# hoivb612/neural

Measured on AMD Instinct MI355X. Metric: decode tokens/sec + prefill TFLOPS, Llama-2-7B int4-g128 at 1/2/4/8 MI355X, higher is better.
Workload: dtype f16; 1 GPU; Llama-2-7B int4-g128 sym decode linear stack, M=1 (32 x [QKV, O, gate/up+SiLU*mul, down] + lm_head), fp32 activations; group_size=128, batch=1, tp=1, parallelism=tp1, hip_graph=True

## Files before the change

neural_amd/bestla.py:

```python
import ctypes as C

import numpy as np

from ._lib import check, last_error, lib

F32, F16, BF16 = 32, 16, 16 | (1 << 16)
S8, S4, S2 = 8 | 0x100, 4 | 0x100, 2 | 0x100
COMP_UNDEF, COMP_F32, COMP_BF16, COMP_F16, COMP_INT8 = 0, 1, 2, 3, 4
ACT_F32, ACT_F16, ACT_BF16 = 0, 1, 2
EPI_NONE, EPI_BIAS, EPI_SILU_MUL, EPI_GELU_MUL, EPI_GELU, EPI_ADD_GELU, EPI_SILU, EPI_RES_ADD = range(8)

S1, S3, S5, S6, S7 = 1 | 0x100, 3 | 0x100, 5 | 0x100, 6 | 0x100, 7 | 0x100
F4_E2M1, F4_BNB, F4_NF4 = 4, 4 | (1 << 16), 4 | (2 << 16)
F8_E4M3, F8_E5M2, F8_E8M0 = 8, 8 | (1 << 16), 8 | (3 << 16)
DQ8_BNB = 8 | (4 << 16)
_WEIGHT_DTYPES = {"int4": S4, "int8": S8, "int2": S2, "int1": S1, "int3": S3, "int5": S5, "int6": S6, "int7": S7,
                  "fp4_e2m1": F4_E2M1, "fp4": F4_E2M1, "nf4": F4_NF4, "fp4_bnb": F4_BNB,
                  "fp8_e4m3": F8_E4M3, "fp8": F8_E4M3, "fp8_e5m2": F8_E5M2}
_SCALE_DTYPES = {"fp32": F32, "bf16": BF16, "fp16": F16, "fp8": F8_E8M0}
_COMP = {"int8": COMP_INT8, "bf16": COMP_BF16, "fp16": COMP_F16, "fp32": COMP_F32, "auto": COMP_UNDEF}
BITS = {S4: 4, S2: 2, S8: 8, S1: 1, S3: 3, S5: 5, S6: 6, S7: 7, F4_E2M1: 4, F4_BNB: 4, F4_NF4: 4, F8_E4M3: 8, F8_E5M2: 8}


def _ptr(a):
# ... 91 lines not shown
    return out


def split(blob, axis, rank, world, unit=1):
    L = lib()
    size = L.nad_blob_split(_ptr(blob), axis, rank, world, unit, None, 0)
    if not size:
        raise RuntimeError(f"nad_blob_split failed: {last_error()}")
    out = _aligned_buffer(size)
    if L.nad_blob_split(_ptr(blob), axis, rank, world, unit, _ptr(out), size) != size:
        raise RuntimeError(f"nad_blob_split failed: {last_error()}")
    return out


def split_range(blob, axis, rank, world, unit=1):
    b, e = C.c_int(0), C.c_int(0)
    check(lib().nad_split_range(_ptr(blob), axis, rank, world, unit, C.byref(b), C.byref(e)), "nad_split_range")
    return b.value, e.value


KERNELS = {1: "woq_gemv_m1_kernel", 2: "woq_gemv_kernel", 3: "woq_skinny_kernel", 4: "woq_i8_kernel",
           5: "woq_gemm3_kernel", 6: "woq_gemm4_kernel", 7: "woq_gemm2_kernel", 8: "woq_gemm_kernel",
           9: "woq_gemm7_kernel", 10: "woq_mid_kernel"}


def plan_forward(bits, n, k, group_size=128, scale_dtype="fp16", asym=False, m=1, act="fp32"):
    o = np.zeros(6, np.int64)
    st = {"fp32": 0, "bf16": 1, "fp16": 2}[scale_dtype]
    at = {"fp32": 0, "fp16": 1, "bf16": 2}[act]
    r = lib().nad_plan_forward(bits, n, k, group_size, st, int(asym), m, at, _ptr(o), 6)
    if r != 6:
        raise RuntimeError(f"nad_plan_forward failed: {last_error()}")
    return dict(kernel=KERNELS.get(int(o[0]), str(int(o[0]))), grid=int(o[1]), threads=int(o[2]), ksplit=int(o[3]),
                fold=bool(o[4] & 1), ksw=bool(o[4] & 2), launches=int(o[5]))


def _torch():
    import torch
    if not torch.cuda.is_available():
        raise RuntimeError("neural_amd device ops need a ROCm GPU (torch.cuda.is_available() is False)")
    return torch


def _stream(stream=None):
    torch = _torch()
    s = stream if stream is not None else torch.cuda.current_stream()
    return C.c_void_p(s.cuda_stream)


_ACT = {}


def _act_code(t):
    torch = _torch()
    if not _ACT:
        _ACT.update({torch.float32: ACT_F32, torch.float16: ACT_F16, torch.bfloat16: ACT_BF16})
    if t.dtype not in _ACT:
        raise TypeError(f"activation dtype {t.dtype} not supported (float32/float16/bfloat16)")
    return _ACT[t.dtype]


class DeviceWeight:

    def __init__(self, blob=None, device=None, stream=None, _desc=None, _mem=None):
        torch = _torch()
        L = lib()
        self.desc = (C.c_uint8 * L.bestla_device_storage_size())()
# ... 49 lines not shown
            raise RuntimeError(last_error())
        blocks = np.ascontiguousarray(blocks, dtype=np.uint8)
        assert blocks.size == n * (k // 32) * bb, (blocks.size, n, k, bb)
        need = L.nad_gguf_device_size(int(type), n, k)
        if not need:
            raise RuntimeError(last_error())
        mem = torch.empty(need, dtype=torch.uint8, device=device or "cuda")
        desc = (C.c_uint8 * L.bestla_device_storage_size())()
        check(L.nad_gguf_device_load(int(type), _ptr(blocks), n, k, desc, _ptr(mem), need, _stream(stream)),
              "nad_gguf_device_load")
        return cls(_desc=desc, _mem=mem)

    def forward(self, x, out=None, epilogue=EPI_NONE, bias=None, residual=None, stream=None):
        torch = _torch()
        m, k = x.shape
        assert k == self.k, (k, self.k)
        if out is None:
            out = torch.empty((m, self.n), dtype=torch.float32, device=x.device)
        bias_ld = 0 if bias is None or bias.dim() == 1 else bias.stride(0)
        check(lib().nad_device_forward(_ptr(x), _act_code(x), self.desc, _ptr(out), m, self.n, k, x.stride(0),
                                       out.stride(0), epilogue, _ptr(bias), bias_ld, _ptr(residual),
                                       residual.stride(0) if residual is not None else 0, _stream(stream)),
              "nad_device_forward")
        return out

    __call__ = forward

    def plan(self, m, act="fp32"):
        o = np.zeros(6, np.int64)
        at = {"fp32": 0, "fp16": 1, "bf16": 2}[act]
        if lib().nad_plan_weight(self.desc, m, at, _ptr(o), 6) != 6:
            raise RuntimeError(f"nad_plan_weight failed: {last_error()}")
        return dict(kernel=KERNELS.get(int(o[0]), str(int(o[0]))), grid=int(o[1]), threads=int(o[2]),
                    ksplit=int(o[3]), fold=bool(o[4] & 1), ksw=bool(o[4] & 2), launches=int(o[5]))

    def set_compute(self, mode):
        check(lib().nad_device_set_compute(self.desc, -1 if mode is None else int(mode)), "nad_device_set_compute")
        return self

    @property
    def compute(self):
        return lib().nad_device_get_compute(self.desc)

    def unpack(self, stream=None):
        out = np.zeros((self.k, self.n), np.float32)
        check(lib().nad_device_unpack_fp32(self.desc, _ptr(out), _stream(stream)), "nad_device_unpack_fp32")
        return out


COMPUTE_FP, COMPUTE_INT8 = 0, 1
GGUF_Q4_0, GGUF_Q4_1, GGUF_Q5_0, GGUF_Q5_1, GGUF_Q8_0 = 2, 3, 6, 7, 8


def set_compute_mode(mode):
    L = lib()
    prev = L.nad_get_compute_mode()
    check(L.nad_set_compute_mode(int(mode)), "nad_set_compute_mode")
    return prev


def get_compute_mode():
    return lib().nad_get_compute_mode()


def set_thread_compute_mode(mode):
    check(lib().nad_set_thread_compute_mode(-1 if mode is None else int(mode)), "nad_set_thread_compute_mode")

# ... 115 lines not shown
```

neural_amd/csrc/capi.hip:

```cpp
#include <hip/hip_runtime.h>

#include <atomic>
#include <cmath>
#include <climits>
#include <cstdarg>
#include <cstdio>
#include <cstdlib>
#include <cstring>
#include <mutex>
#include <string>
#include <unordered_map>
#include <vector>

#include "../../include/neural_amd.h"
#include "btla_format.h"
#include "woq_kernels.h"

using namespace nad;

static thread_local std::string g_err;
static void set_err(const char* fmt, ...) {
  char buf[512];
  va_list ap;
  va_start(ap, fmt);
  vsnprintf(buf, sizeof(buf), fmt, ap);
  va_end(ap);
  g_err = buf;
}
static void report(const char* where) { fprintf(stderr, "neural_amd: %s: %s\n", where, g_err.c_str()); }
#define HIP_OK(expr)                                                           \
  do {                                                                         \
    hipError_t e_ = (expr);                                                    \
    if (e_ != hipSuccess) {                                                    \
      set_err("%s failed: %s", #expr, hipGetErrorString(e_));                  \
      return -1;                                                               \
    }                                                                          \
  } while (0)

extern "C" const char* nad_last_error(void) { return g_err.c_str(); }
extern "C" void nad_clear_error(void) { g_err.clear(); }

static int env_int(const char* name, int def) {
  const char* v = getenv(name);
  return (v && *v) ? atoi(v) : def;
}

struct Knobs {
  int gemv_grid, gemv_waves, gemv_lean, gemv_spw, gemv_disable, gemv_dual, gemv_nst;
  int compute_int8;
  int gemm2_disable, gemm4_all, gemm4_disable, ffn_f32, gemm_kernel, gemm7_bm, splitk_disable;
  int gemm3_stagger, gemm4_fold_all, gemm4_fold, gemm4_ksw;
  int mid_min_m, mid_max_m, mid_ks, mid_xcd, mid_wide, gemm_xcd, gemm7_model, gemm7_fuse;
  int host_cache_mb;
};
static Knobs read_knobs() {
  Knobs k{};
  k.gemv_grid = env_int("NAD_GEMV_GRID", 0);
  k.gemv_waves = env_int("NAD_GEMV_WAVES", 0);
  k.gemv_nst = env_int("NAD_GEMV_NST", 0);
  k.gemv_lean = env_int("NAD_GEMV_LEAN", 1);
  k.gemv_dual = env_int("NAD_GEMV_DUAL", 1);
  k.gemv_spw = env_int("NAD_GEMV_SPW", 4);
  k.gemv_disable = env_int("NAD_GEMV_DISABLE", 0);
  k.compute_int8 = env_int("NAD_COMPUTE_INT8", 0);
  k.gemm2_disable = env_int("NAD_GEMM2_DISABLE", 0);
  k.gemm4_all = env_int("NAD_GEMM4_ALL", 0);
  k.gemm4_disable = env_int("NAD_GEMM4_DISABLE", 0);
  k.ffn_f32 = env_int("NAD_FFN_F32", 0);
  k.gemm_kernel = env_int("NAD_GEMM_KERNEL", 7);
  k.gemm7_bm = env_int("NAD_GEMM7_BM", 0);
  k.splitk_disable = env_int("NAD_SPLITK_DISABLE", 0);
  k.gemm3_stagger = env_int("NAD_GEMM3_STAGGER", 1);
  k.gemm4_fold_all = env_int("NAD_GEMM4_FOLD_ALL", 1);
  k.gemm4_fold = env_int("NAD_GEMM4_FOLD", 1);
  k.gemm4_ksw = env_int("NAD_GEMM4_KSW", 2);
  k.mid_max_m = env_int("NAD_MID_MAX_M", 64);
  k.mid_ks = env_int("NAD_MID_KS", 0);
  k.mid_xcd = env_int("NAD_MID_XCD", 1);
  k.mid_wide = env_int("NAD_MID_WIDE", 2);
  k.gemm_xcd = env_int("NAD_GEMM_XCD", 1);
  k.gemm7_fuse = env_int("NAD_GEMM7_FUSE", 1);
  k.gemm7_model = env_int("NAD_GEMM7_MODEL", 2);
  k.mid_min_m = env_int("NAD_MID_MIN_M", 0);
  k.host_cache_mb = env_int("NAD_HOST_CACHE_MB", 64 * 1024);
  return k;
}
static Knobs g_knobs = read_knobs();
static const Knobs& knobs() { return g_knobs; }
extern "C" void nad_reload_knobs(void) { g_knobs = read_knobs(); }

struct NadPlan {
  int kernel = 0, grid = 0, block = 0, ksplit = 1, fold = 0, launches = 0;
};
// ... 329 lines not shown
  a.act_t = act_t;
  a.dual = (epi == kEpiSiluMul || epi == kEpiGeluMul) ? 1 : 0;
  a.nt = w0.nt;
  a.ng = w0.ng;
  a.bs = w0.blocksize;
  a.tpg_mask = tpg == 0 ? 0x7fffffff : tpg - 1;
  a.tpg_shift = tpg == 0 ? 31 : __builtin_ctz(unsigned(tpg));
  a.scale_t = w0.scale_t;
  a.asym = w0.asym;
  a.epi = epi;
  a.shuffle = w0.shuffle;
  a.a_fast = (vec_aligned(act, lda, act_t) && w0.shuffle == nullptr && k % 8 == 0) ? 1 : 0;
  a.res = res;
  a.ld_res = ld_res;
  a.aux = aux;
  a.ld_aux = ld_aux;
  int stripes = 0;
  for (int i = 0; i < 4; i++) a.stripe_base[i] = INT_MAX;
  for (int i = 0; i < nw; i++) {
    a.w[i] = view(*ws[i], outs[i], ldos[i], bias, bias_ld);
    a.stripe_base[i] = stripes;
    stripes += ws[i]->ns;
  }
  for (int i = nw; i < 3; i++) a.w[i] = a.w[0];
  a.units = a.dual ? ws[0]->ns : stripes;
  const Knobs& kn = knobs();
  grid = std::max(1, std::min(a.units, device_cus()));
  if (kn.gemv_grid > 0) grid = std::min(a.units, kn.gemv_grid);
  waves = gemv_waves(w0.bits, w0.nt, w0.ng, w0.blocksize);
  if (kn.gemv_waves > 0) waves = std::min(gpt > 1 ? 8 : 16, kn.gemv_waves);
  a.dq_mask = 0x000F000Fu;
  a.dq_magic = 0x64006400u;
  a.m1_nst = kn.gemv_nst;
  a.u_q = a.units / grid;
  a.u_r = a.units % grid;
  a.lean = kn.gemv_lean;
  if (single_op)
    gemv_lean_slices(a, w0.bits, &waves, kn.gemv_waves > 0 ? 4 : 2);
  if (kn.gemv_spw != 4 && a.lean_spw == 4) a.lean_spw = 2;
  const size_t lds = gemv_lds_layout(a, w0.bits, waves, grid);
  if (lds > 160 * 1024) return 0;
  const int esz = act_t == kActF32 ? 4 : 2;
  if (uint64_t(m) * lda * esz >= (1ull << 30)) return 0;
  for (int i = 0; i < nw; i++)
    if (uint64_t(ws[i]->ns) * ws[i]->nt * 1024 >= (1ull << 30)) return 0;
  gpt_out = gpt;
  (void)lds;
  return 1;
}

static int try_gemv(const void* act, int act_t, int lda, int m, int k, int nw, const DeviceWeight* const* ws,
                    float* const* outs, const int* ldos, int epi, const float* bias, int bias_ld, const float* res,
                    int ld_res, float* aux, int ld_aux, hipStream_t st) {
  if (knobs().gemv_disable) return 0;
  GemvArgs a{};
  int waves = 0, grid = 0, gpt = 0;
  if (!prepare_gemv(a, waves, grid, gpt, act, act_t, lda, m, k, nw, ws, outs, ldos, epi, bias, bias_ld, res, ld_res,
                    aux, ld_aux))
    return 0;
  const size_t lds = gemv_lds_layout(a, ws[0]->bits, waves, grid);
  hipError_t e = planned(gemv_uses_m1(a, ws[0]->bits, waves) ? NAD_KERNEL_GEMV_M1 : NAD_KERNEL_GEMV, grid, waves * 64)
                     ? hipSuccess
                     : launch_gemv(a, ws[0]->bits, waves, grid, lds, st);
  if (e != hipSuccess) {
    set_err("gemv kernel launch failed: %s", hipGetErrorString(e));
    return -1;
  }
  return 1;
}

static bool int8_compute(const DeviceWeight& w);
static int gguf_act_quant(const DeviceWeight& w);
static int run_i8(const void* act, int act_t, int lda, int m, int k, int nw, const DeviceWeight* const* ws,
                  float* const* outs, const int* ldos, bool dual, int epi, const float* bias, int bias_ld,
                  const float* res, int ld_res, const float* aux, int ld_aux, hipStream_t st);

static int run_skinny(const void* act, int act_t, int lda, int m, int k, int nw, const DeviceWeight* const* ws,
                      float* const* outs, const int* ldos, int epi, const float* bias, int bias_ld, const float* res,
                      int ld_res, float* aux, int ld_aux, hipStream_t st) {
  if (nw > 1) {
    bool mixed = false;
    for (int i = 1; i < nw; i++)
      mixed |= int8_compute(*ws[i]) != int8_compute(*ws[0]) || gguf_act_quant(*ws[i]) != gguf_act_quant(*ws[0]);
    if (mixed) {
      if (epi == kEpiSiluMul || epi == kEpiGeluMul) {
        set_err("gate/up weights of one FFN must resolve to the same arithmetic (nad_device_set_compute)");
        return -1;
      }
      for (int i = 0; i < nw; i++)
        if (run_skinny(act, act_t, lda, m, k, 1, ws + i, outs + i, ldos + i, epi, bias, bias_ld, res, ld_res, aux,
                       ld_aux, st))
          return -1;
      return 0;
    }
// ... 2145 lines not shown
```

neural_amd/csrc/woq_gemv.hip:

```cpp
#include <hip/hip_runtime.h>

#include <climits>
#include <cstdint>

#include "woq_device.h"
#include "woq_kernels.h"

namespace nad {

#ifdef NAD_PHASE_TRACE
constexpr int kTraceSlots = 8, kTraceMaxWg = 16384;
__device__ unsigned long long nad_trace_buf[kTraceSlots][kTraceMaxWg];
#define NAD_TRACE(slot)                                                                       \
  do {                                                                                        \
    if (threadIdx.x == 0 && blockIdx.x < kTraceMaxWg) nad_trace_buf[slot][blockIdx.x] = wall_clock64(); \
  } while (0)
#define NAD_TRACE_MAX(slot)                                                                               \
  do {                                                                                                    \
    if ((threadIdx.x & 63) == 0 && blockIdx.x < kTraceMaxWg)                                              \
      atomicMax(&nad_trace_buf[slot][blockIdx.x], (unsigned long long)wall_clock64());                    \
  } while (0)
#else
#define NAD_TRACE(slot) \
  do {                  \
// ... 731 lines not shown
        float s0 = 0.f, s1 = 0.f, s2 = 0.f, s3 = 0.f;
#pragma unroll
        for (int w = 0; w < 16; w += 4)
          if (w < full) {
            s0 += t[w];
            s1 += t[w + 1];
            s2 += t[w + 2];
            s3 += t[w + 3];
          }
#pragma unroll
        for (int w = 0; w < 16; w++)
          if (w >= full && w < nwl) s0 += t[w];
        y[h] = (s0 + s1) + (s2 + s3);
      }
    }
    emit(p, nn, y);
  }
  NAD_TRACE(3);
}

template <int BITS, int GPT, int AT, bool ASYM, int KSN, int SPW, bool BATCH, int NST, int ST>
__global__ __launch_bounds__((m1_max_threads<GPT, KSN>())) void woq_gemv_m1_kernel(GemvArgs a) {
  m1_body<BITS, GPT, AT, ASYM, KSN, SPW, BATCH, NST, ST>(a, int(blockIdx.x));
}

template <int B1, int G1, int K1, int B2, int G2, int K2, int AT>
__global__ __launch_bounds__(1024) void woq_gemv_m1_dual_kernel(GemvArgs a, GemvArgs b, int ga) {
  if (int(blockIdx.x) < ga)
    m1_body<B1, G1, AT, false, K1, 1, false, NAD_M1_DUAL_NST>(a, int(blockIdx.x));
  else
    m1_body<B2, G2, AT, false, K2, 1, false, NAD_M1_DUAL_NST>(b, int(blockIdx.x) - ga);
}

template <int BITS, int HILO, int GPT, bool ASYM, int NST>
static hipError_t gemv_launch5(const GemvArgs& a, dim3 g, dim3 b, size_t lds, hipStream_t st) {
  auto k = woq_gemv_kernel<BITS, HILO, GPT, ASYM, NST>;
  static bool attr_set = false;
  if (!attr_set) {
    hipError_t e = hipFuncSetAttribute(reinterpret_cast<const void*>(k), hipFuncAttributeMaxDynamicSharedMemorySize,
                                       160 * 1024);
    if (e != hipSuccess) return e;
    attr_set = true;
  }
  hipLaunchKernelGGL(k, g, b, lds, st, a);
  return hipGetLastError();
}
template <int BITS, int HILO, int GPT, bool ASYM>
static hipError_t gemv_launch4(const GemvArgs& a, dim3 g, dim3 b, size_t lds, hipStream_t st) {
  const int nsl = (a.nt + KS - 1) / KS, waves = int(b.x / 64);
  const int spw = (a.u_q + (a.u_r ? 1 : 0)) * (a.dual ? 2 : 1) * ((nsl + waves - 1) / waves);
  const int nst = a.m1_nst == 1 ? 1 : (a.m1_nst == 3 ? 3 : (spw <= 2 ? 1 : 3));
  return nst == 1 ? gemv_launch5<BITS, HILO, GPT, ASYM, 1>(a, g, b, lds, st)
                  : gemv_launch5<BITS, HILO, GPT, ASYM, 3>(a, g, b, lds, st);
}

template <int BITS, int GPT, int AT, bool ASYM, int KSN, int SPW, int NST, int ST>
static hipError_t gemv_m1_launch6(const GemvArgs& a, dim3 g, dim3 b, size_t lds, hipStream_t st) {
  auto k = woq_gemv_m1_kernel<BITS, GPT, AT, ASYM, KSN, SPW, false, NST, ST>;
  static bool attr_set = false;
  if (!attr_set) {
    hipError_t e = hipFuncSetAttribute(reinterpret_cast<const void*>(k), hipFuncAttributeMaxDynamicSharedMemorySize,
                                       160 * 1024);
    if (e != hipSuccess) return e;
    attr_set = true;
  }
  hipLaunchKernelGGL(k, g, b, lds, st, a);
// ... 8 lines not shown
  if (a.batch) {
    auto kb = woq_gemv_m1_kernel<BITS, GPT, AT, ASYM, KSN, SPW, true, NAD_M1_BATCH_NST, ST>;
    static bool attr_b = false;
    if (!attr_b) {
      hipError_t e = hipFuncSetAttribute(reinterpret_cast<const void*>(kb), hipFuncAttributeMaxDynamicSharedMemorySize,
                                         160 * 1024);
      if (e != hipSuccess) return e;
      attr_b = true;
    }
    hipLaunchKernelGGL(kb, g, b, lds, st, a);
    return hipGetLastError();
  }
  const int spw = m1_stages_per_wave(a, KSN, int(b.x / 64));
  const int nst = a.m1_nst == 1 || a.m1_nst == 2 ? a.m1_nst : (spw >= 7 || (KSN == 1 && spw >= 4) ? 2 : 1);
  return nst == 1 ? gemv_m1_launch6<BITS, GPT, AT, ASYM, KSN, SPW, 1, ST>(a, g, b, lds, st)
                  : gemv_m1_launch6<BITS, GPT, AT, ASYM, KSN, SPW, 2, ST>(a, g, b, lds, st);
}
#ifndef NAD_INT2_ST
#define NAD_INT2_ST 1
#endif
template <int BITS, int GPT, int AT, bool ASYM, int ST = -1>
static hipError_t gemv_m1_launch4(const GemvArgs& a, dim3 g, dim3 b, size_t lds, hipStream_t st) {
  if constexpr (BITS == 2 && ST < 0 && NAD_INT2_ST) {
    if (a.scale_t == kScaleF32) return gemv_m1_launch4<BITS, GPT, AT, ASYM, kScaleF32>(a, g, b, lds, st);
    if (a.scale_t == kScaleBF16) return gemv_m1_launch4<BITS, GPT, AT, ASYM, kScaleBF16>(a, g, b, lds, st);
    return gemv_m1_launch4<BITS, GPT, AT, ASYM, kScaleF16>(a, g, b, lds, st);
  } else {
    if (a.lean_ks == 1) return gemv_m1_launch5<BITS, GPT, AT, ASYM, 1, 1, ST>(a, g, b, lds, st);
    if (a.lean_ks == 2) return gemv_m1_launch5<BITS, GPT, AT, ASYM, 2, 1, ST>(a, g, b, lds, st);
    return a.lean_spw == 4 ? gemv_m1_launch5<BITS, GPT, AT, ASYM, KS, 4, ST>(a, g, b, lds, st)
                           : gemv_m1_launch5<BITS, GPT, AT, ASYM, KS, 2, ST>(a, g, b, lds, st);
  }
}
template <int BITS, int GPT>
static hipError_t gemv_m1_launch2(const GemvArgs& a, dim3 g, dim3 b, size_t lds, hipStream_t st) {
  if (a.act_t == kActF32) return a.asym ? gemv_m1_launch4<BITS, GPT, kActF32, true>(a, g, b, lds, st)
                                        : gemv_m1_launch4<BITS, GPT, kActF32, false>(a, g, b, lds, st);
  if (a.act_t == kActF16) return a.asym ? gemv_m1_launch4<BITS, GPT, kActF16, true>(a, g, b, lds, st)
                                        : gemv_m1_launch4<BITS, GPT, kActF16, false>(a, g, b, lds, st);
  return a.asym ? gemv_m1_launch4<BITS, GPT, kActBF16, true>(a, g, b, lds, st)
                : gemv_m1_launch4<BITS, GPT, kActBF16, false>(a, g, b, lds, st);
}
#if !defined(GEMV_PART) || GEMV_PART == 1
hipError_t gemv_m1_launch_b2(const GemvArgs& a, int gpt, dim3 g, dim3 b, size_t lds, hipStream_t st) {
  if (gpt == 1) return gemv_m1_launch2<2, 1>(a, g, b, lds, st);
  if (gpt == 2) return gemv_m1_launch2<2, 2>(a, g, b, lds, st);
  if (gpt == 4 && !a.asym) return a.act_t == kActF32 ? gemv_m1_launch4<2, 4, kActF32, false>(a, g, b, lds, st)
                                 : (a.act_t == kActF16 ? gemv_m1_launch4<2, 4, kActF16, false>(a, g, b, lds, st)
                                                       : gemv_m1_launch4<2, 4, kActBF16, false>(a, g, b, lds, st));
  return hipErrorInvalidValue;
}
#else
hipError_t gemv_m1_launch_b2(const GemvArgs& a, int gpt, dim3 g, dim3 b, size_t lds, hipStream_t st);
#endif
#if !defined(GEMV_PART) || GEMV_PART == 0
static hipError_t gemv_m1_launch(const GemvArgs& a, int bits, int gpt, dim3 g, dim3 b, size_t lds, hipStream_t st) {
  if (bits == 4) {
    if (gpt == 1) return gemv_m1_launch2<4, 1>(a, g, b, lds, st);
    if (gpt == 2) return gemv_m1_launch2<4, 2>(a, g, b, lds, st);
    return hipErrorInvalidValue;
  }
  return gemv_m1_launch_b2(a, gpt, g, b, lds, st);
}

template <int BITS, int HILO>
static hipError_t gemv_launch2(const GemvArgs& a, int gpt, dim3 g, dim3 b, size_t lds, hipStream_t st) {
// ... 55 lines not shown
  const int nsl = (a.nt + ks - 1) / ks;
  if (nsl > 16 || nsl <= *waves) return;
  if (!lean_ok(a, bits, *waves)) return;
  a.lean_ks = ks;
  a.lean_spw = 1;
  if (!lean_ok(a, bits, nsl)) {
    a.lean_ks = KS;
    a.lean_spw = 2;
    return;
  }
  *waves = nsl;
}

int gemv_groups_per_tile(int bits, int nt, int ng, int bs, int* tpg) {
  const int KT = bits == 4 ? 128 : (bits == 2 ? 256 : 64);
  if (ng == 1) {
    *tpg = 0;
    return 1;
  }
  if (bs % KT == 0) {
    *tpg = bs / KT;
    return (*tpg & (*tpg - 1)) == 0 ? 1 : 0;
  }
  if (KT % bs == 0 && bs % 32 == 0) {
    *tpg = 1;
    const int g = KT / bs;
    return (g == 2 || g == 4) ? g : 0;
  }
  return 0;
}

bool gemv_uses_m1(const GemvArgs& a, int bits, int waves) { return lean_ok(a, bits, waves); }

bool gemv_dual_ok(const GemvArgs& a, int bits_a, const GemvArgs& b, int bits_b, int waves) {
  int tpg = 0;
  const int ga = gemv_groups_per_tile(bits_a, a.nt, a.ng, a.bs, &tpg), gb = gemv_groups_per_tile(bits_b, b.nt, b.ng, b.bs, &tpg);
  const bool pair = bits_a == 2 && bits_b == 4 && ((ga == 4 && gb == 2) || (ga == 2 && gb == 1));
  return pair && !a.asym && !b.asym && a.lean_ks == 1 && b.lean_ks == 2 && a.act_t == kActF32 && b.act_t == kActF32 &&
         waves == 16 && lean_ok(a, bits_a, waves) && lean_ok(b, bits_b, waves);
}

hipError_t launch_gemv_dual(const GemvArgs& a, const GemvArgs& b, int ga, int gb, int waves, size_t lds,
                            hipStream_t stream) {
  int tpg = 0;
  const int g1 = gemv_groups_per_tile(2, a.nt, a.ng, a.bs, &tpg);
  auto go = [&](auto k) -> hipError_t {
    static bool attr = false;
    if (!attr) {
      hipError_t e = hipFuncSetAttribute(reinterpret_cast<const void*>(k), hipFuncAttributeMaxDynamicSharedMemorySize,
                                         160 * 1024);
      if (e != hipSuccess) return e;
      attr = true;
    }
    hipLaunchKernelGGL(k, dim3(ga + gb), dim3(waves * 64), lds, stream, a, b, ga);
    return hipGetLastError();
  };
  if (g1 == 4) return go(woq_gemv_m1_dual_kernel<2, 4, 1, 4, 2, 2, kActF32>);
  return go(woq_gemv_m1_dual_kernel<2, 2, 1, 4, 1, 2, kActF32>);
}

hipError_t launch_gemv_batch(const GemvArgs& a, int bits, int waves, int grid, size_t lds, hipStream_t stream) {
  int tpg = 0;
  const int gpt = gemv_groups_per_tile(bits, a.nt, a.ng, a.bs, &tpg);
  if (gpt == 0 || !a.batch || a.batch_wpp <= 0 || !lean_ok(a, bits, waves)) return hipErrorInvalidValue;
  return gemv_m1_launch(a, bits, gpt, dim3(grid), dim3(waves * 64), lds, stream);
}

hipError_t launch_gemv(const GemvArgs& a, int bits, int waves, int grid, size_t lds, hipStream_t stream) {
  const int hilo = a.act_t == kActF16 ? 0 : (a.M <= 8 ? 1 : 2);
  int tpg = 0;
  const int gpt = gemv_groups_per_tile(bits, a.nt, a.ng, a.bs, &tpg);
  if (gpt == 0) return hipErrorInvalidValue;
  dim3 g(grid), b(waves * 64);
  if (lean_ok(a, bits, waves)) return gemv_m1_launch(a, bits, gpt, g, b, lds, stream);
  if (bits == 4) return gemv_launch1<4>(a, hilo, gpt, g, b, lds, stream);
  if (bits == 2) return gemv_launch1<2>(a, hilo, gpt, g, b, lds, stream);
  return gemv_launch1<8>(a, hilo, gpt, g, b, lds, stream);
}

#endif

}

#if defined(NAD_PHASE_TRACE) && (!defined(GEMV_PART) || GEMV_PART == 0)
extern "C" int nad_trace_clock_khz() {
  int dev = 0, khz = 0;
  if (hipGetDevice(&dev) != hipSuccess) return -1;
  if (hipDeviceGetAttribute(&khz, hipDeviceAttributeWallClockRate, dev) != hipSuccess) return -1;
  return khz;
}

extern "C" int nad_trace_fetch(void* host, size_t bytes, int clear, int grid_filter) {
  (void)grid_filter;
  const size_t n = sizeof(nad::nad_trace_buf) < bytes ? sizeof(nad::nad_trace_buf) : bytes;
  if (hipDeviceSynchronize() != hipSuccess) return -1;
  if (host && hipMemcpyFromSymbol(host, HIP_SYMBOL(nad::nad_trace_buf), n) != hipSuccess) return -1;
  if (clear) {
    void* p = nullptr;
    if (hipGetSymbolAddress(&p, HIP_SYMBOL(nad::nad_trace_buf)) != hipSuccess) return -1;
    if (hipMemset(p, 0, sizeof(nad::nad_trace_buf)) != hipSuccess) return -1;
    if (hipDeviceSynchronize() != hipSuccess) return -1;
  }
  return 0;
}
#endif
```

neural_amd/csrc/woq_kernels.h:

```cpp
#pragma once
#include <hip/hip_runtime.h>

#include <algorithm>
#include <cstdint>

#include "woq_layout.h"

namespace nad {

enum ActType : int { kActF32 = 0, kActF16 = 1, kActBF16 = 2 };

struct RepackArgs {
  const uint8_t* src_q;
  const void* src_s;
  const int8_t* src_z;
  int ntile, packrow, kpad, cstep;
  int src_bits;
  uint64_t nel;
  int raw;
  int src_e8m0;
  int bits, n, k, ns, nt, ng, scale_t, kmajor;
  uint32_t* dst_tiles;
  void* dst_scales;
  int8_t* dst_zps;
// ... 75 lines not shown
  const void* A;
  int lda, M, K;
  int act_t;
  int dual;
  int units;
  int stripe_base[4];
  int nt, ng, bs;
  int tpg_mask;
  int tpg_shift;
  int scale_t;
  int asym;
  int epi;
  int a_fast;
  const int32_t* shuffle;
  const float* res;
  int ld_res;
  float* aux;
  int ld_aux;
  int part_off;
  uint32_t dq_mask;
  uint32_t dq_magic;
  int nwa;
  int norm;
  float norm_eps;
  const float* norm_w;
  int u_q, u_r;
  int lean;
  int lean_ks;
  int lean_spw;
  SkinnyWeight w[3];
  const GemvBatchEnt* batch;
  int batch_wpp;
  int m1_nst;
};

hipError_t launch_repack(const RepackArgs& a, hipStream_t stream);
hipError_t launch_skinny(const SkinnyArgs& a, int bits, int act_t, int waves_per_wg, int stripes, int ch,
                         hipStream_t stream);
hipError_t launch_gemm(const GemmArgs& a, int bits, int act_t, hipStream_t stream);
hipError_t launch_gemm2(const GemmArgs& a, const _Float16* A16, int lda16, hipStream_t stream);
hipError_t launch_gemm3(const GemmArgs& a, const _Float16* A16, int lda16, hipStream_t stream);
int gemm4_mode(int bits, int blocksize, int ng, int kpad, bool asym);

struct QuantU8Args {
  const void* A;
  int lda, M, K, bs, ng;
  const int32_t* shuffle;
  int8_t* aq;
  int ldq, kp;
  float2* sa;
  uint8_t* q_u8;
  int ldu;
  float* s_out;
  uint8_t* z_out;
  float* red_out;
  int ld_scale;
};
struct I8Args {
  const int8_t* aq;
  int ldq;
  int a_signed;
  const float2* sa;
  int M, K;
  const uint16_t* red;
  int red_ld;
  int scale_t;
// ... 21 lines not shown
  int s_ld, s_st;
  const uint16_t* mins;
  const uint16_t* scales;
  float qbias;
  int ns, ng, kmajor;
  GemmArgs g;
};
constexpr int kMinTermSmallM = 16;
constexpr size_t kMinTermSmallLds = 65536;
hipError_t launch_q4_0_repack(const uint8_t* src, int n, int k, const DeviceWeight& w, hipStream_t stream);
hipError_t launch_gguf_repack(int type, const uint8_t* src, int n, int k, const DeviceWeight& w, hipStream_t stream);
hipError_t launch_q8_1_quant(const Q81Args& a, int act_t, hipStream_t stream);
hipError_t launch_block_sums(const void* A, int act_t, int lda, int M, int K, float* S, hipStream_t stream);
hipError_t launch_min_term(const MinTermArgs& a, int act_t, hipStream_t stream);
hipError_t launch_min_term_tiled(const MinTermArgs& a, hipStream_t stream);
hipError_t launch_q8_0_quant(const Q80Args& a, int act_t, hipStream_t stream);
hipError_t launch_quant_u8(const QuantU8Args& a, int act_t, hipStream_t stream);
hipError_t launch_i8(const I8Args& a, int bits, hipStream_t stream);
hipError_t launch_gemm4(const GemmArgs& a, int bits, const _Float16* A16, int lda16, hipStream_t stream);
bool gemm7_ok(int bits, int blocksize, int fold_ok);
hipError_t launch_gemm7(const GemmArgs& a, int bits, int bm, const _Float16* A16, int lda16, hipStream_t stream);
void mid_geometry(int bits, int gpt, int act_t, int rf, int wide, int* s, int* nw, int* spw);
int mid_lds_bytes(int rf, int s, int nw);
hipError_t launch_gemm_mid(const GemmArgs& a, int bits, int gpt, int act_t, int rf, int s, int grid, hipStream_t stream);
hipError_t launch_splitk_reduce(const GemmArgs& a, hipStream_t stream);
hipError_t launch_cvt_act(const void* A, int act_t, int lda, int M, int K, int Kp, const int32_t* shuffle,
                          _Float16* out, hipStream_t stream);
int gemv_groups_per_tile(int bits, int nt, int ng, int bs, int* tpg);
size_t gemv_lds_layout(GemvArgs& a, int bits, int waves, int grid);
int gemv_waves(int bits, int nt, int ng, int bs);
void gemv_lean_slices(GemvArgs& a, int bits, int* waves, int ks_pref);
hipError_t launch_gemv(const GemvArgs& a, int bits, int waves, int grid, size_t lds, hipStream_t stream);
bool gemv_uses_m1(const GemvArgs& a, int bits, int waves);
bool gemv_dual_ok(const GemvArgs& a, int bits_a, const GemvArgs& b, int bits_b, int waves);
hipError_t launch_gemv_dual(const GemvArgs& a, const GemvArgs& b, int ga, int gb, int waves, size_t lds,
                            hipStream_t stream);
hipError_t launch_gemv_batch(const GemvArgs& a, int bits, int waves, int grid, size_t lds, hipStream_t stream);

}
```

Baseline: 971.8 tokens/s.

## Add specialized compact-args M=1 GEMV kernel with per-weight-count templates

Adds a new woq_gemv_m1s_kernel for M=1 decode that takes a compact GemvM1Args struct, templated on the number of fused weights (1, gate/up pair with SiLU*mul, or 3 for QKV) and on a 16-wave fixed-reduction variant. The launcher tries this path first when lean M=1 applies, and falls back to the existing m1 kernel otherwise. The intent is to cut kernel-argument size, runtime branching and register pressure in the hot decode GEMVs. It adds many template instantiations, which raises compile time and binary size, and relies on the new selection logic matching the old plan's coverage.

```diff
diff --git a/neural_amd/bestla.py b/neural_amd/bestla.py
--- a/neural_amd/bestla.py
+++ b/neural_amd/bestla.py
@@ -147,7 +147,7 @@
     if r != 6:
         raise RuntimeError(f"nad_plan_forward failed: {last_error()}")
     return dict(kernel=KERNELS.get(int(o[0]), str(int(o[0]))), grid=int(o[1]), threads=int(o[2]), ksplit=int(o[3]),
-                fold=bool(o[4] & 1), ksw=bool(o[4] & 2), launches=int(o[5]))
+                fold=bool(o[4] & 1), ksw=bool(o[4] & 2), m1_spec=bool(o[4] & 4), launches=int(o[5]))
 
 
 def _torch():
@@ -263,7 +263,7 @@
         if lib().nad_plan_weight(self.desc, m, at, _ptr(o), 6) != 6:
             raise RuntimeError(f"nad_plan_weight failed: {last_error()}")
         return dict(kernel=KERNELS.get(int(o[0]), str(int(o[0]))), grid=int(o[1]), threads=int(o[2]),
-                    ksplit=int(o[3]), fold=bool(o[4] & 1), ksw=bool(o[4] & 2), launches=int(o[5]))
+                    ksplit=int(o[3]), fold=bool(o[4] & 1), ksw=bool(o[4] & 2), m1_spec=bool(o[4] & 4), launches=int(o[5]))
 
     def set_compute(self, mode):
         check(lib().nad_device_set_compute(self.desc, -1 if mode is None else int(mode)), "nad_device_set_compute")
diff --git a/neural_amd/csrc/capi.hip b/neural_amd/csrc/capi.hip
--- a/neural_amd/csrc/capi.hip
+++ b/neural_amd/csrc/capi.hip
@@ -46,7 +46,7 @@
 }
 
 struct Knobs {
-  int gemv_grid, gemv_waves, gemv_lean, gemv_spw, gemv_disable, gemv_dual, gemv_nst;
+  int gemv_grid, gemv_waves, gemv_lean, gemv_spw, gemv_disable, gemv_dual, gemv_nst, gemv_m1_spec;
   int compute_int8;
   int gemm2_disable, gemm4_all, gemm4_disable, ffn_f32, gemm_kernel, gemm7_bm, splitk_disable;
   int gemm3_stagger, gemm4_fold_all, gemm4_fold, gemm4_ksw;
@@ -59,6 +59,7 @@
   k.gemv_waves = env_int("NAD_GEMV_WAVES", 0);
   k.gemv_nst = env_int("NAD_GEMV_NST", 0);
   k.gemv_lean = env_int("NAD_GEMV_LEAN", 1);
+  k.gemv_m1_spec = env_int("NAD_GEMV_M1_SPEC", 1);
   k.gemv_dual = env_int("NAD_GEMV_DUAL", 1);
   k.gemv_spw = env_int("NAD_GEMV_SPW", 4);
   k.gemv_disable = env_int("NAD_GEMV_DISABLE", 0);
@@ -454,6 +455,7 @@
   a.dq_mask = 0x000F000Fu;
   a.dq_magic = 0x64006400u;
   a.m1_nst = kn.gemv_nst;
+  a.m1_spec = kn.gemv_m1_spec;
   a.u_q = a.units / grid;
   a.u_r = a.units % grid;
   a.lean = kn.gemv_lean;
@@ -481,7 +483,8 @@
                     aux, ld_aux))
     return 0;
   const size_t lds = gemv_lds_layout(a, ws[0]->bits, waves, grid);
-  hipError_t e = planned(gemv_uses_m1(a, ws[0]->bits, waves) ? NAD_KERNEL_GEMV_M1 : NAD_KERNEL_GEMV, grid, waves * 64)
+  hipError_t e = planned(gemv_uses_m1(a, ws[0]->bits, waves) ? NAD_KERNEL_GEMV_M1 : NAD_KERNEL_GEMV, grid, waves * 64, 1,
+                         t_plan && gemv_uses_m1s(a, ws[0]->bits, waves) ? 4 : 0)
                      ? hipSuccess
                      : launch_gemv(a, ws[0]->bits, waves, grid, lds, st);
   if (e != hipSuccess) {
diff --git a/neural_amd/csrc/woq_gemv.hip b/neural_amd/csrc/woq_gemv.hip
--- a/neural_amd/csrc/woq_gemv.hip
+++ b/neural_amd/csrc/woq_gemv.hip
@@ -787,6 +787,275 @@
     m1_body<B2, G2, AT, false, K2, 1, false, NAD_M1_DUAL_NST>(b, int(blockIdx.x) - ga);
 }
 
+template <int NWT>
+struct M1Sel {
+  int w, s;
+  __device__ __forceinline__ M1Sel(const GemvM1Args<NWT>& a, int v) {
+    if constexpr (NWT == 1) {
+      w = 0;
+      s = v;
+    } else if constexpr (NWT == 2) {
+      w = v & 1;
+      s = v >> 1;
+    } else {
+      w = (v >= a.sb1 ? 1 : 0) + (v >= a.sb2 ? 1 : 0);
+      s = v - (w == 0 ? 0 : (w == 1 ? a.sb1 : a.sb2));
+    }
+  }
+};
+template <int NWT, class T>
+__device__ __forceinline__ T m1_pick(int w, const T (&x)[3]) {
+  if constexpr (NWT == 1) return x[0];
+  else if constexpr (NWT == 2) return w == 0 ? x[0] : x[1];
+  else return sel3(w, x[0], x[1], x[2]);
+}
+#define NAD_M1_FIELD(args, wi, f) \
+  m1_pick<NWT>(wi, {args.w[0].f, args.w[NWT > 1 ? 1 : 0].f, args.w[NWT > 2 ? 2 : 0].f})
+
+template <int NWT, bool ASYM>
+__device__ __forceinline__ void m1s_cursor_stripe(const GemvM1Args<NWT>& a, StageCursor& c, int v, bool on) {
+  const M1Sel<NWT> vs(a, v);
+  c.s = vs.s;
+  const void* const tp[3] = {a.w[0].tiles, a.w[NWT > 1 ? 1 : 0].tiles, a.w[NWT > 2 ? 2 : 0].tiles};
+  const void* const sp[3] = {a.w[0].scales, a.w[NWT > 1 ? 1 : 0].scales, a.w[NWT > 2 ? 2 : 0].scales};
+  const int tb[3] = {a.w[0].tiles_bytes, a.w[NWT > 1 ? 1 : 0].tiles_bytes, a.w[NWT > 2 ? 2 : 0].tiles_bytes};
+  const int sb[3] = {a.w[0].scales_bytes, a.w[NWT > 1 ? 1 : 0].scales_bytes, a.w[NWT > 2 ? 2 : 0].scales_bytes};
+  c.rt = rsrc(m1_pick<NWT>(vs.w, tp), on ? m1_pick<NWT>(vs.w, tb) : 0);
+  c.rs = rsrc(m1_pick<NWT>(vs.w, sp), on ? m1_pick<NWT>(vs.w, sb) : 0);
+  if constexpr (ASYM) {
+    const void* const zp[3] = {a.w[0].zps, a.w[NWT > 1 ? 1 : 0].zps, a.w[NWT > 2 ? 2 : 0].zps};
+    const int zb[3] = {a.w[0].zps_bytes, a.w[NWT > 1 ? 1 : 0].zps_bytes, a.w[NWT > 2 ? 2 : 0].zps_bytes};
+    c.rz = rsrc(m1_pick<NWT>(vs.w, zp), on ? m1_pick<NWT>(vs.w, zb) : 0);
+  } else {
+    c.rz = c.rs;
+  }
+}
+
+template <int GPT, bool ASYM, int KSN, int NWT>
+__device__ __forceinline__ void m1s_load_stage(const GemvM1Args<NWT>& a, StageRegs<GPT, KSN>& S, StageCursor& c, int nv,
+                                               int nsl, int wave, int NW, int v0, int lane, int vs) {
+  const bool on = c.j < nv;
+  const int nt = a.nt, ng = a.ng;
+  const int t0 = c.q * KSN;
+  const int tb = (c.s * nt + t0) * 1024;
+  const int rowb = a.scale_t == kScaleF32 ? 64 : 32;
+#pragma unroll
+  for (int i = 0; i < KSN; i++) {
+    const bool live = on && t0 + i < nt;
+    S.b[i] = __builtin_bit_cast(u4_t, __builtin_amdgcn_raw_buffer_load_b128(c.rt, (live ? tb + i * 1024 : kOOB) + lane * 16, 0, NAD_TILE_AUX));
+#pragma unroll
+    for (int g = 0; g < GPT; g++) {
+      const int grp = GPT == 1 ? ((t0 + i) >> a.tpg_shift) : (t0 + i) * GPT + g;
+      const bool gl = live && (GPT == 1 || grp < ng);
+      const int row = c.s * ng + grp;
+      S.sc[i][g] = __builtin_amdgcn_raw_buffer_load_b32(c.rs, (gl ? row * rowb : kOOB) + vs, 0, 0);
+      if constexpr (ASYM)
+        S.zp[i][g] = int(int8_t(__builtin_amdgcn_raw_buffer_load_b8(c.rz, (gl ? row * 16 : kOOB) + (lane & 15), 0, 0)));
+      else
+        S.zp[i][g] = 0;
+    }
+  }
+  if (on) {
+    c.q += NW;
+    if (c.q >= nsl) {
+      c.q = wave;
+      c.j++;
+      m1s_cursor_stripe<NWT, ASYM>(a, c, v0 + c.j, c.j < nv);
+    }
+  }
+}
+
+template <int BITS, int GPT, int AT, bool ASYM, int KSN, int SPW, int NST, int ST, int NWT, bool L16>
+__global__ __launch_bounds__((m1_max_threads<GPT, KSN>())) void woq_gemv_m1s_kernel(GemvM1Args<NWT> a) {
+  extern __shared__ __attribute__((aligned(16))) char smem[];
+  static_assert(NWT >= 1 && NWT <= 3, "1 weight, the {gate, up} pair, or 3 weights");
+  constexpr int KT = BITS == 4 ? 128 : 256, SPT = KT / 32, SPG = SPT / GPT;
+  constexpr int RB = lean_row_bytes(BITS, KSN);
+  constexpr int UNITS = KSN * KT / 8;
+  constexpr int UPL = UNITS >= 64 ? UNITS / 64 : 1;
+  constexpr bool PART = UNITS < 64;
+  constexpr int BIAS = BITS == 4 ? 8 : 2;
+  constexpr int ESZ = AT == kActF32 ? 4 : 2;
+  constexpr bool HL = AT != kActF16;
+  constexpr int VPU = NWT == 2 ? 2 : 1;
+  const int lane = threadIdx.x & 63;
+  const int wave = __builtin_amdgcn_readfirstlane(int(threadIdx.x >> 6));
+  const int NW = L16 ? 16 : a.nw;
+  const int nsl = a.nsl;
+  const bool ulane = !PART || lane < UNITS;
+  NAD_TRACE(0);
+  const int bid = int(blockIdx.x);
+  const int u0 = bid * a.u_q + min(bid, a.u_r);
+  const int nu = a.u_q + (bid < a.u_r ? 1 : 0);
+  const int v0 = u0 * VPU, nv = nu * VPU;
+  const bool idle = !L16 && wave >= nsl;
+  float* part = reinterpret_cast<float*>(smem + a.part_off);
+
+  const auto ra = rsrc(a.A, a.a_bytes);
+  uint4 x[SPW * UPL][2];
+#pragma unroll
+  for (int j = 0; j < SPW * UPL; j++) {
+    const int q = wave + (j / UPL) * NW, k = q * (KSN * KT) + ((j % UPL) * 64 + lane) * 8;
+    const int off = ulane ? k * ESZ : kOOB;
+    x[j][0] = __builtin_bit_cast(uint4, __builtin_amdgcn_raw_buffer_load_b128(ra, off, 0, 0));
+    if constexpr (ESZ == 4) x[j][1] = __builtin_bit_cast(uint4, __builtin_amdgcn_raw_buffer_load_b128(ra, off + 16, 0, 0));
+  }
+  const int vs = a.scale_t == kScaleF32 ? (lane & 15) * 4 : (lane & 14) * 2;
+  StageCursor lc;
+  lc.j = idle ? nv : 0;
+  lc.q = wave;
+  m1s_cursor_stripe<NWT, ASYM>(a, lc, v0, lc.j < nv);
+  StageRegs<GPT, KSN> S[NST];
+  m1s_load_stage<GPT, ASYM, KSN, NWT>(a, S[0], lc, nv, nsl, wave, NW, v0, lane, vs);
+  NAD_TRACE(4);
+
+  char* wrow = smem + wave * lean_wave_lds(BITS, KSN, SPW);
+#pragma unroll
+  for (int u = 0; u < UPL; u++)
+    if (ulane) *reinterpret_cast<uint4*>(wrow + (u * 64 + lane) * 16) = make_uint4(0u, 0u, 0u, 0u);
+#pragma unroll
+  for (int j = 0; j < SPW * UPL; j++) {
+    if (!ulane) break;
+    h8_t hi, lo;
+    if constexpr (AT == kActF16) {
+      hi = __builtin_bit_cast(h8_t, x[j][0]);
+    } else {
+      float f[8];
+      unit_to_f32(AT, x[j][0], x[j][1], f);
+#pragma unroll
+      for (int e = 0; e < 8; e++) {
+        hi[e] = _Float16(f[e]);
+        lo[e] = _Float16(f[e] - float(hi[e]));
+      }
+    }
+    char* row = wrow + RB + (j / UPL) * 2 * RB + ((j % UPL) * 64 + lane) * 16;
+    *reinterpret_cast<h8_t*>(row) = hi;
+    if constexpr (HL) *reinterpret_cast<h8_t*>(row + RB) = lo;
+  }
+#pragma unroll
+  for (int i = 1; i < NST; i++) m1s_load_stage<GPT, ASYM, KSN, NWT>(a, S[i], lc, nv, nsl, wave, NW, v0, lane, vs);
+  NAD_TRACE(1);
+
+  const int m = lane & 15, kq = lane >> 4;
+  const bool isrow = m == 0 || (HL && m == 8);
+  const char* abase = wrow + (isrow ? (m == 0 ? RB : 2 * RB) : 0) + kq * 16;
+  const int slice_step = isrow ? 2 * RB : 0;
+  const int ssh = a.scale_t == kScaleF32 ? 0 : (lane & 1) * 16;
+  Dq4 dq;
+  dq.m0 = __builtin_amdgcn_readfirstlane(a.dq_mask);
+  dq.m1 = dq.m0 << 4;
+  dq.mag = __builtin_amdgcn_readfirstlane(a.dq_magic);
+  dq.s16 = splat(1.f / 16.f);
+  const h2_t zc0 = splat(-(1024.f + BIAS)), zc1 = splat(-(64.f + BIAS));
+
+  f4_t acc = {0.f, 0.f, 0.f, 0.f};
+  int cj = idle ? nv : 0, cq = wave, cs = 0;
+
+  auto compute_stage = [&](const StageRegs<GPT, KSN>& S) {
+    if (cj >= nv) return;
+    const char* ab = abase + cs * slice_step;
+    f4_t accg[KSN];
+#pragma unroll
+    for (int d = 0; d < SPT; d++) {
+      const int g = GPT == 1 ? 0 : d / SPG;
+#pragma unroll
+      for (int i = 0; i < KSN; i++) {
+        h8_t bf;
+        if constexpr (BITS == 4) {
+          if constexpr (ASYM) {
+            const float z = float(S.zp[i][g]);
+            bf = dequant4(S.b[i][d], dq, zc0 - splat(z), zc1 - splat(z));
+          } else {
+            bf = dequant4(S.b[i][d], dq, zc0, zc1);
+          }
+        } else {
+          bf = BITS == 2 ? dequant2_step(S.b[i], d, BIAS + S.zp[i][g])
+                         : dequant_step<BITS>(S.b[i], d, zp_const(BIAS + S.zp[i][g]));
+        }
+        const h8_t af = *reinterpret_cast<const h8_t*>(ab + i * KT * 2 + d * 64);
+        accg[i] = __builtin_amdgcn_mfma_f32_16x16x32_f16(af, bf, d % SPG == 0 ? f4_t{0.f, 0.f, 0.f, 0.f} : accg[i],
+                                                         0, 0, 0);
+      }
+      if ((d + 1) % SPG == 0) {
+#pragma unroll
+        for (int i = 0; i < KSN; i++) acc += accg[i] * scale_to_f32<ST>(S.sc[i][g], a.scale_t, ssh);
+      }
+    }
+    cq += NW;
+    cs++;
+    if (cq >= nsl) {
+      float r = acc[0];
+      if constexpr (HL) {
+        r += __shfl_down(r, 32, 64);
+      }
+      if (lane < 16) part[(size_t(cj) * 16 + lane) * NW + wave] = r;
+      acc = f4_t{0.f, 0.f, 0.f, 0.f};
+      cq = wave;
+      cs = 0;
+      cj++;
+    }
+  };
+
+  while (cj < nv) {
+#pragma unroll
+    for (int i = 0; i < NST; i++) {
+      compute_stage(S[i]);
+      m1s_load_stage<GPT, ASYM, KSN, NWT>(a, S[i], lc, nv, nsl, wave, NW, v0, lane, vs);
+    }
+  }
+  NAD_TRACE_MAX(2);
+  __syncthreads();
+
+  const int nout = nu * 16;
+  for (int o = threadIdx.x; o < nout; o += NW * 64) {
+    const int p = o >> 4, nn = o & 15;
+    float y[VPU];
+#pragma unroll
+    for (int h = 0; h < VPU; h++) {
+      if constexpr (L16) {
+        const float4* ps = reinterpret_cast<const float4*>(part + (size_t(p * VPU + h) * 16 + nn) * 16);
+        const float4 t0 = ps[0], t1 = ps[1], t2 = ps[2], t3 = ps[3];
+        const float s0 = ((t0.x + t1.x) + t2.x) + t3.x, s1 = ((t0.y + t1.y) + t2.y) + t3.y;
+        const float s2 = ((t0.z + t1.z) + t2.z) + t3.z, s3 = ((t0.w + t1.w) + t2.w) + t3.w;
+        y[h] = (s0 + s1) + (s2 + s3);
+      } else {
+        const int nwl = min(NW, nsl);
+        const float* ps = part + (size_t(p * VPU + h) * 16 + nn) * NW;
+        float t[16];
+#pragma unroll
+        for (int w = 0; w < 16; w++) t[w] = ps[min(w, nwl - 1)];
+        const int full = nwl & ~3;
+        float s0 = 0.f, s1 = 0.f, s2 = 0.f, s3 = 0.f;
+#pragma unroll
+        for (int w = 0; w < 16; w += 4)
+          if (w < full) {
+            s0 += t[w];
+            s1 += t[w + 1];
+            s2 += t[w + 2];
+            s3 += t[w + 3];
+          }
+#pragma unroll
+        for (int w = 0; w < 16; w++)
+          if (w >= full && w < nwl) s0 += t[w];
+        y[h] = (s0 + s1) + (s2 + s3);
+      }
+    }
+    const M1Sel<NWT> vsel(a, v0 + p * VPU);
+    const int wsel = NWT == 2 ? 0 : vsel.w;
+    const int n = vsel.s * 16 + nn;
+    if (n >= NAD_M1_FIELD(a, wsel, n)) continue;
+    float* out = NAD_M1_FIELD(a, wsel, out);
+    if constexpr (NWT == 2) {
+      const float t1 = silu_f(y[0]);
+      if (a.aux) a.aux[n] = t1;
+      out[n] = t1 * y[VPU - 1];
+    } else {
+      out[n] = y[0];
+    }
+  }
+  NAD_TRACE(3);
+}
+
 template <int BITS, int HILO, int GPT, bool ASYM, int NST>
 static hipError_t gemv_launch5(const GemvArgs& a, dim3 g, dim3 b, size_t lds, hipStream_t st) {
   auto k = woq_gemv_kernel<BITS, HILO, GPT, ASYM, NST>;
@@ -861,6 +1130,141 @@
                            : gemv_m1_launch5<BITS, GPT, AT, ASYM, KS, 2, ST>(a, g, b, lds, st);
   }
 }
+template <int NWT>
+static GemvM1Args<NWT> m1s_args(const GemvArgs& a, int ksn, int waves) {
+  GemvM1Args<NWT> c{};
+  const int esz = a.act_t == kActF32 ? 4 : 2, ssz = a.scale_t == kScaleF32 ? 4 : 2;
+  c.A = a.A;
+  c.a_bytes = a.K * esz;
+  c.nsl = (a.nt + ksn - 1) / ksn;
+  c.u_q = a.u_q;
+  c.u_r = a.u_r;
+  c.nt = a.nt;
+  c.ng = a.ng;
+  c.tpg_shift = a.tpg_shift;
+  c.scale_t = a.scale_t;
+  c.nw = waves;
+  c.part_off = a.part_off;
+  c.dq_mask = a.dq_mask;
+  c.dq_magic = a.dq_magic;
+  c.sb1 = a.stripe_base[1];
+  c.sb2 = a.stripe_base[2];
+  for (int i = 0; i < NWT; i++) {
+    const SkinnyWeight& w = a.w[i];
+    c.w[i].tiles = w.tiles;
+    c.w[i].scales = w.scales;
+    c.w[i].zps = w.zps;
+    c.w[i].tiles_bytes = w.ns * a.nt * 1024;
+    c.w[i].scales_bytes = w.ns * a.ng * 16 * ssz;
+    c.w[i].zps_bytes = w.ns * a.ng * 16;
+    c.w[i].n = w.n;
+    c.w[i].out = w.out;
+  }
+  c.aux = a.aux;
+  return c;
+}
+template <int BITS, int GPT, int AT, bool ASYM, int KSN, int SPW, int NST, int ST, int NWT, bool L16>
+static hipError_t m1s_go(const GemvArgs& a, dim3 g, dim3 b, size_t lds, hipStream_t st) {
+  auto k = woq_gemv_m1s_kernel<BITS, GPT, AT, ASYM, KSN, SPW, NST, ST, NWT, L16>;
+  static bool attr_set = false;
+  if (!attr_set) {
+    hipError_t e = hipFuncSetAttribute(reinterpret_cast<const void*>(k), hipFuncAttributeMaxDynamicSharedMemorySize,
+                                       160 * 1024);
+    if (e != hipSuccess) return e;
+    attr_set = true;
+  }
+  const GemvM1Args<NWT> c = m1s_args<NWT>(a, KSN, int(b.x / 64));
+  hipLaunchKernelGGL(k, g, b, lds, st, c);
+  return hipGetLastError();
+}
+static int m1s_nwt(const GemvArgs& a) {
+  if (a.batch || !a.m1_spec) return 0;
+  if (a.dual) return a.epi == kEpiSiluMul ? 2 : 0;
+  if (a.epi != kEpiNone) return 0;
+  const int nw = 1 + (a.stripe_base[1] != INT_MAX ? 1 : 0) + (a.stripe_base[2] != INT_MAX ? 1 : 0);
+  return nw == 1 || nw == 3 ? nw : 0;
+}
+template <int BITS, int GPT, int AT, bool ASYM, int ST>
+static bool m1s_launch3(const GemvArgs& a, dim3 g, dim3 b, size_t lds, hipStream_t st, hipError_t* e) {
+  const int nwt = m1s_nwt(a), waves = int(b.x / 64), ks = lean_ks(a);
+  if (nwt == 0) return false;
+  const int nsl = (a.nt + ks - 1) / ks;
+  const bool l16 = waves == 16 && nsl >= 16;
+  const int spw = m1_stages_per_wave(a, ks, waves);
+  const int nst = a.m1_nst == 1 || a.m1_nst == 2 ? a.m1_nst : (spw >= 7 || (ks == 1 && spw >= 4) ? 2 : 1);
+#define NAD_M1S(KSN, SPW, NST, NWT, L16)                                                         \
+  do {                                                                                           \
+    if (e) *e = m1s_go<BITS, GPT, AT, ASYM, KSN, SPW, NST, ST, NWT, L16>(a, g, b, lds, st);      \
+    return true;                                                                                 \
+  } while (0)
+#define NAD_M1S_NARROW(KSN)                               \
+  do {                                                    \
+    if (nst == 1) {                                       \
+      if (nwt == 1 && l16) NAD_M1S(KSN, 1, 1, 1, true);   \
+      if (nwt == 1) NAD_M1S(KSN, 1, 1, 1, false);         \
+      if (nwt == 2 && l16) NAD_M1S(KSN, 1, 1, 2, true);   \
+      if (nwt == 2) NAD_M1S(KSN, 1, 1, 2, false);         \
+      if (nwt == 3 && l16) NAD_M1S(KSN, 1, 1, 3, true);   \
+      if (nwt == 3) NAD_M1S(KSN, 1, 1, 3, false);         \
+    } else if (nwt == 1) {                                \
+      if (l16) NAD_M1S(KSN, 1, 2, 1, true);               \
+      NAD_M1S(KSN, 1, 2, 1, false);                       \
+    }                                                     \
+    return false;                                         \
+  } while (0)
+  if (ks == 1) NAD_M1S_NARROW(1);
+  if (ks == 2) NAD_M1S_NARROW(2);
+  if (l16 || (GPT != 1 && waves > 8)) return false;
+  if (lean_spw(a) == 4) {
+    if (nwt == 1 && nst == 1) NAD_M1S(KS, 4, 1, 1, false);
+    return false;
+  }
+  if (nst == 1) {
+    if (nwt == 1) NAD_M1S(KS, 2, 1, 1, false);
+    if (nwt == 2) NAD_M1S(KS, 2, 1, 2, false);
+    NAD_M1S(KS, 2, 1, 3, false);
+  }
+  if (nwt == 1) NAD_M1S(KS, 2, 2, 1, false);
+  return false;
+#undef NAD_M1S_NARROW
+#undef NAD_M1S
+}
+#if !defined(GEMV_PART) || GEMV_PART == 2
+bool gemv_m1s_launch_b4(const GemvArgs& a, int gpt, dim3 g, dim3 b, size_t lds, hipStream_t st, hipError_t* e) {
+  if (gpt == 1) {
+    if (a.act_t == kActF32) return a.asym ? m1s_launch3<4, 1, kActF32, true, -1>(a, g, b, lds, st, e)
+                                          : m1s_launch3<4, 1, kActF32, false, -1>(a, g, b, lds, st, e);
+    if (a.act_t == kActF16) return a.asym ? m1s_launch3<4, 1, kActF16, true, -1>(a, g, b, lds, st, e)
+                                          : m1s_launch3<4, 1, kActF16, false, -1>(a, g, b, lds, st, e);
+    return a.asym ? m1s_launch3<4, 1, kActBF16, true, -1>(a, g, b, lds, st, e)
+                  : m1s_launch3<4, 1, kActBF16, false, -1>(a, g, b, lds, st, e);
+  }
+  if (gpt == 2 && a.act_t == kActF32)
+    return a.asym ? m1s_launch3<4, 2, kActF32, true, -1>(a, g, b, lds, st, e)
+                  : m1s_launch3<4, 2, kActF32, false, -1>(a, g, b, lds, st, e);
+  return false;
+}
+#else
+bool gemv_m1s_launch_b4(const GemvArgs& a, int gpt, dim3 g, dim3 b, size_t lds, hipStream_t st, hipError_t* e);
+#endif
+#if !defined(GEMV_PART) || GEMV_PART == 3
+template <int GPT>
+static bool m1s_launch_b2g(const GemvArgs& a, dim3 g, dim3 b, size_t lds, hipStream_t st, hipError_t* e) {
+  if (a.scale_t == kScaleF32) return m1s_launch3<2, GPT, kActF32, false, NAD_INT2_ST ? kScaleF32 : -1>(a, g, b, lds, st, e);
+  if (a.scale_t == kScaleBF16) return m1s_launch3<2, GPT, kActF32, false, NAD_INT2_ST ? kScaleBF16 : -1>(a, g, b, lds, st, e);
+  return m1s_launch3<2, GPT, kActF32, false, NAD_INT2_ST ? kScaleF16 : -1>(a, g, b, lds, st, e);
+}
+bool gemv_m1s_launch_b2(const GemvArgs& a, int gpt, dim3 g, dim3 b, size_t lds, hipStream_t st, hipError_t* e) {
+  if (a.asym || a.act_t != kActF32) return false;
+  if (gpt == 1) return m1s_launch_b2g<1>(a, g, b, lds, st, e);
+  if (gpt == 2) return m1s_launch_b2g<2>(a, g, b, lds, st, e);
+  if (gpt == 4) return m1s_launch_b2g<4>(a, g, b, lds, st, e);
+  return false;
+}
+#else
+bool gemv_m1s_launch_b2(const GemvArgs& a, int gpt, dim3 g, dim3 b, size_t lds, hipStream_t st, hipError_t* e);
+#endif
+
 template <int BITS, int GPT>
 static hipError_t gemv_m1_launch2(const GemvArgs& a, dim3 g, dim3 b, size_t lds, hipStream_t st) {
   if (a.act_t == kActF32) return a.asym ? gemv_m1_launch4<BITS, GPT, kActF32, true>(a, g, b, lds, st)
@@ -982,6 +1386,14 @@
 
 bool gemv_uses_m1(const GemvArgs& a, int bits, int waves) { return lean_ok(a, bits, waves); }
 
+bool gemv_uses_m1s(const GemvArgs& a, int bits, int waves) {
+  int tpg = 0;
+  const int gpt = gemv_groups_per_tile(bits, a.nt, a.ng, a.bs, &tpg);
+  if (!lean_ok(a, bits, waves)) return false;
+  return bits == 4 ? gemv_m1s_launch_b4(a, gpt, dim3(1), dim3(waves * 64), 0, nullptr, nullptr)
+                   : gemv_m1s_launch_b2(a, gpt, dim3(1), dim3(waves * 64), 0, nullptr, nullptr);
+}
+
 bool gemv_dual_ok(const GemvArgs& a, int bits_a, const GemvArgs& b, int bits_b, int waves) {
   int tpg = 0;
   const int ga = gemv_groups_per_tile(bits_a, a.nt, a.ng, a.bs, &tpg), gb = gemv_groups_per_tile(bits_b, b.nt, b.ng, b.bs, &tpg);
@@ -1022,7 +1434,12 @@
   const int gpt = gemv_groups_per_tile(bits, a.nt, a.ng, a.bs, &tpg);
   if (gpt == 0) return hipErrorInvalidValue;
   dim3 g(grid), b(waves * 64);
-  if (lean_ok(a, bits, waves)) return gemv_m1_launch(a, bits, gpt, g, b, lds, stream);
+  if (lean_ok(a, bits, waves)) {
+    hipError_t e = hipSuccess;
+    if (bits == 4 ? gemv_m1s_launch_b4(a, gpt, g, b, lds, stream, &e) : gemv_m1s_launch_b2(a, gpt, g, b, lds, stream, &e))
+      return e;
+    return gemv_m1_launch(a, bits, gpt, g, b, lds, stream);
+  }
   if (bits == 4) return gemv_launch1<4>(a, hilo, gpt, g, b, lds, stream);
   if (bits == 2) return gemv_launch1<2>(a, hilo, gpt, g, b, lds, stream);
   return gemv_launch1<8>(a, hilo, gpt, g, b, lds, stream);
diff --git a/neural_amd/csrc/woq_kernels.h b/neural_amd/csrc/woq_kernels.h
--- a/neural_amd/csrc/woq_kernels.h
+++ b/neural_amd/csrc/woq_kernels.h
@@ -131,6 +131,32 @@
   const GemvBatchEnt* batch;
   int batch_wpp;
   int m1_nst;
+  int m1_spec;
+};
+
+struct GemvM1Weight {
+  const void* tiles;
+  const void* scales;
+  const int8_t* zps;
+  int tiles_bytes, scales_bytes, zps_bytes;
+  int n;
+  float* out;
+};
+template <int NWS>
+struct GemvM1Args {
+  const void* A;
+  int a_bytes;
+  int nsl;
+  int u_q, u_r;
+  int nt, ng;
+  int tpg_shift;
+  int scale_t;
+  int nw;
+  int part_off;
+  uint32_t dq_mask, dq_magic;
+  int sb1, sb2;
+  GemvM1Weight w[NWS];
+  float* aux;
 };
 
 hipError_t launch_repack(const RepackArgs& a, hipStream_t stream);
@@ -218,6 +244,7 @@
 void gemv_lean_slices(GemvArgs& a, int bits, int* waves, int ks_pref);
 hipError_t launch_gemv(const GemvArgs& a, int bits, int waves, int grid, size_t lds, hipStream_t stream);
 bool gemv_uses_m1(const GemvArgs& a, int bits, int waves);
+bool gemv_uses_m1s(const GemvArgs& a, int bits, int waves);
 bool gemv_dual_ok(const GemvArgs& a, int bits_a, const GemvArgs& b, int bits_b, int waves);
 hipError_t launch_gemv_dual(const GemvArgs& a, const GemvArgs& b, int ga, int gb, int waves, size_t lds,
                             hipStream_t stream);
```

Measured after the change: 1028 tokens/s, median of 6. 1.06x the previous value.
